# Rikorose/DeepFilterNet

Hardware: NVIDIA H100
Metric: 48kHz audio-sec/sec (batched enhance) (higher is better)
Workload: dtype f32 (bf16x3 tensor-core contractions, fp32 accumulate; DSP and gates IEEE fp32)

## Files before the change

deepfilternet_b200/csrc/dfb_ptx.cuh:

```cuda
#pragma once
#include <cuda.h>
#include <cuda_bf16.h>
#include <stdint.h>

namespace dfb {

__device__ __forceinline__ uint32_t smem_u32(const void *p) { return (uint32_t)__cvta_generic_to_shared(p); }

__device__ __forceinline__ void mbar_init(uint64_t *bar, uint32_t count) {
    asm volatile("mbarrier.init.shared::cta.b64 [%0], %1;" ::"r"(smem_u32(bar)), "r"(count));
}

__device__ __forceinline__ void mbar_expect_tx(uint64_t *bar, uint32_t bytes) {
    asm volatile("mbarrier.arrive.expect_tx.shared::cta.b64 _, [%0], %1;" ::"r"(smem_u32(bar)), "r"(bytes) : "memory");
}

__device__ __forceinline__ void mbar_wait(uint64_t *bar, uint32_t parity) {
    asm volatile(
        "{\n\t"
        ".reg .pred p;\n\t"
        "WAIT_%=:\n\t"
        "mbarrier.try_wait.parity.shared::cta.b64 p, [%0], %1;\n\t"
        "@p bra DONE_%=;\n\t"
        "bra WAIT_%=;\n\t"
// ... 46 lines not shown
__device__ __forceinline__ void warp_mma_sw128_k64(uint32_t a_hi, uint32_t a_lo, uint32_t b_hi, uint32_t b_lo, int m0, int n0,
                                                   float (&acc)[MT][8][4]) {
    const int lane = threadIdx.x & 31, mat = lane >> 3, rr = lane & 7;
#pragma unroll
    for (int ks = 0; ks < 4; ks++) {
        uint32_t ah[MT][4], al[MT][4];
#pragma unroll
        for (int mt = 0; mt < MT; mt++) {
            const int r = m0 + 16 * mt + rr + ((mat & 1) << 3);
            const uint32_t o = sw128_off(r, 2 * ks + (mat >> 1));
            ldsm_x4(a_hi + o, ah[mt]);
            ldsm_x4(a_lo + o, al[mt]);
        }
#pragma unroll
        for (int np = 0; np < 4; np++) {
            const int n = n0 + 16 * np + rr + ((mat >> 1) << 3);
            const uint32_t o = sw128_off(n, 2 * ks + (mat & 1));
            uint32_t bh[4], bl[4];
            ldsm_x4(b_hi + o, bh);
            ldsm_x4(b_lo + o, bl);
#pragma unroll
            for (int mt = 0; mt < MT; mt++) {
                mma_bf16x3(acc[mt][2 * np], ah[mt], al[mt], bh[0], bh[1], bl[0], bl[1]);
                mma_bf16x3(acc[mt][2 * np + 1], ah[mt], al[mt], bh[2], bh[3], bl[2], bl[3]);
            }
        }
    }
}

__device__ __forceinline__ void mbar_arrive(uint64_t *bar) {
    asm volatile("mbarrier.arrive.shared::cta.b64 _, [%0];" ::"r"(smem_u32(bar)) : "memory");
}



__device__ __forceinline__ void bf16x2_split(float x0, float x1, uint32_t &hi, uint32_t &lo) {
    __nv_bfloat162 h = __floats2bfloat162_rn(x0, x1);
    const float2 hf = __bfloat1622float2(h);
    __nv_bfloat162 l = __floats2bfloat162_rn(x0 - hf.x, x1 - hf.y);
    hi = *reinterpret_cast<uint32_t *>(&h);
    lo = *reinterpret_cast<uint32_t *>(&l);
}

__device__ __forceinline__ float4 lds128(uint32_t a) {
    float4 v;
    asm volatile("ld.shared.v4.f32 {%0, %1, %2, %3}, [%4];" : "=f"(v.x), "=f"(v.y), "=f"(v.z), "=f"(v.w) : "r"(a));
    return v;
}

__device__ __forceinline__ void sts128(uint32_t a, float4 v) {
    asm volatile("st.shared.v4.f32 [%0], {%1, %2, %3, %4};" ::"r"(a), "f"(v.x), "f"(v.y), "f"(v.z), "f"(v.w) : "memory");
}

__device__ __forceinline__ void sts64(uint32_t a, uint32_t x, uint32_t y) {
    asm volatile("st.shared.v2.b32 [%0], {%1, %2};" ::"r"(a), "r"(x), "r"(y) : "memory");
}

__device__ __forceinline__ uint32_t lds32(uint32_t a) {
    uint32_t v;
    asm volatile("ld.shared.b32 %0, [%1];" : "=r"(v) : "r"(a));
    return v;
}

__device__ __forceinline__ void mbar_init_a(uint32_t bar, uint32_t count) {
    asm volatile("mbarrier.init.shared::cta.b64 [%0], %1;" ::"r"(bar), "r"(count));
}
// ... 64 lines not shown
```

deepfilternet_b200/csrc/dfb_tc.cu:

```cuda
#include <cooperative_groups.h>
#include <atomic>
#include <map>
#include <mutex>
#include <cuda.h>
#include <cuda_bf16.h>

#include "dfb_common.cuh"
#include "dfb_dwpw.cuh"
#include "dfb_ptx.cuh"

namespace dfb {

constexpr int kBxBM = 128, kBxBN = 128, kBxBK = 64, kBxStages = 3, kBxThreads = 288;
constexpr int kBxBox = 128 * 128;

struct BxSmem {
    alignas(1024) unsigned char x[kBxStages][2][kBxBox];
    alignas(1024) unsigned char w[kBxStages][2][kBxBox];
    alignas(8) uint64_t full[kBxStages];
    uint64_t empty[kBxStages];
};

__global__ void __launch_bounds__(kBxThreads, 1)
k_gemm_bf16x3(const __grid_constant__ CUtensorMap tmXhi, const __grid_constant__ CUtensorMap tmXlo,
              const __grid_constant__ CUtensorMap tmWhi, const __grid_constant__ CUtensorMap tmWlo,
              const float *__restrict__ bias, float *__restrict__ Y, int64_t ldy, int M, int K, int nslices) {
    extern __shared__ __align__(1024) unsigned char tc_smem_raw[];
    BxSmem &sm = *reinterpret_cast<BxSmem *>(((uintptr_t)tc_smem_raw + 1023) & ~uintptr_t(1023));
    const int warp = threadIdx.x >> 5, lane = threadIdx.x & 31;
    const int n0 = (int)(blockIdx.x % nslices) * kBxBN, m0 = (int)(blockIdx.x / nslices) * kBxBM;
    const int nkb = K / kBxBK;
    if (threadIdx.x == 0) {
        for (int s = 0; s < kBxStages; s++) { mbar_init(&sm.full[s], 1); mbar_init(&sm.empty[s], 8); }
        fence_barrier_init();
    }
    __syncthreads();
    if (warp == 8) {
        if (lane == 0) {
            tma_prefetch_desc(&tmXhi); tma_prefetch_desc(&tmXlo); tma_prefetch_desc(&tmWhi); tma_prefetch_desc(&tmWlo);
            for (int kb = 0; kb < nkb; kb++) {
                const int s = kb % kBxStages, n = kb / kBxStages;
                if (n > 0) mbar_wait(&sm.empty[s], (n - 1) & 1);
                mbar_expect_tx(&sm.full[s], 4 * kBxBox);
                tma_load_2d(sm.x[s][0], &tmXhi, kb * kBxBK, m0, &sm.full[s]);
                tma_load_2d(sm.x[s][1], &tmXlo, kb * kBxBK, m0, &sm.full[s]);
                tma_load_2d(sm.w[s][0], &tmWhi, kb * kBxBK, n0, &sm.full[s]);
                tma_load_2d(sm.w[s][1], &tmWlo, kb * kBxBK, n0, &sm.full[s]);
            }
        }
        return;
    }
    const int wm = (warp & 3) * 32, wn = (warp >> 2) * 64;
    float acc[2][8][4];
#pragma unroll
    for (int a = 0; a < 2; a++)
#pragma unroll
        for (int b = 0; b < 8; b++)
#pragma unroll
            for (int c = 0; c < 4; c++) acc[a][b][c] = 0.f;
    for (int kb = 0; kb < nkb; kb++) {
        const int s = kb % kBxStages;
        mbar_wait(&sm.full[s], (kb / kBxStages) & 1);
        warp_mma_sw128_k64<2>(smem_u32(sm.x[s][0]), smem_u32(sm.x[s][1]), smem_u32(sm.w[s][0]), smem_u32(sm.w[s][1]), wm, wn, acc);
        __syncwarp();
        if (lane == 0) mbar_arrive(&sm.empty[s]);
    }
#pragma unroll
    for (int nt = 0; nt < 8; nt++) {
        const int n = n0 + wn + 8 * nt + 2 * (lane & 3);
        const float2 bn = bias ? make_float2(__ldg(bias + n), __ldg(bias + n + 1)) : make_float2(0.f, 0.f);
#pragma unroll
        for (int mt = 0; mt < 2; mt++)
#pragma unroll
            for (int h = 0; h < 2; h++) {
                const int m = m0 + wm + 16 * mt + (lane >> 2) + 8 * h;
                if (m < M)
                    *reinterpret_cast<float2 *>(Y + (int64_t)m * ldy + n) =
                        make_float2(acc[mt][nt][2 * h] + bn.x, acc[mt][nt][2 * h + 1] + bn.y);
            }
    }
}

constexpr int kDxThreads = 256;
constexpr uint32_t kDxW = 32768, kDxRaw = 49152, kDxTail = 64 * 4 + 32;


template <int MODE, int KT, int PATH, int MASK>
__global__ void __launch_bounds__(kDxThreads, 2)
k_dwpw_bx(DwPwParams p, const float *__restrict__ w_sw ) {
    extern __shared__ __align__(1024) unsigned char tc_smem_raw[];
    const uint32_t sb = smem_u32(tc_smem_raw);
    if (sb & 1023u) __trap();
    const int tid = threadIdx.x, warp = tid >> 5, lane = tid & 31;
    const int b = blockIdx.y, t0 = blockIdx.x * p.NF;
    const int nf = min(p.NF, p.T - t0);
    const int R = nf * p.Fout;
    const int tq0 = t0 - (KT - 1);
    const uint32_t fbytes = (uint32_t)p.Fin * kCh * 4;
    const uint32_t raw_in = sb + kDxRaw, raw_path = raw_in + (uint32_t)(p.NF + KT - 1) * fbytes;
    const uint32_t raw_e0 = raw_in + (uint32_t)(p.NF + KT - 1) * fbytes * (PATH ? 2u : 1u);
    const uint32_t obytes = (uint32_t)p.Fout * kCh * 4;
    const uint32_t tail = raw_e0 + (MASK ? (uint32_t)p.NF * obytes : 0u);
    const uint32_t s_bias = tail, bar_raw = tail + 264;
    const uint32_t s_mask = raw_in;
    if (tid == 0) {
        mbar_init_a(bar_raw, 1);
        fence_barrier_init();
        const int ta = max(tq0, 0), tb = t0 + nf;
        mbar_expect_tx_a(bar_raw, (uint32_t)(tb - ta) * fbytes * (PATH ? 2u : 1u) + 2u * kCh * 128u + (MASK ? (uint32_t)nf * obytes : 0u));
        if (MASK)
            for (int t = t0; t < tb; t++)
                bulk_load(raw_e0 + (uint32_t)(t - t0) * obytes, p.mk_e0 + ((int64_t)b * p.T + t) * p.Fout * kCh, obytes, bar_raw);
// ... 672 lines not shown
        if (rc) return rc;
    }
    if (xg == 0 || xg == 1) {
        if (H == 512 && ns == 16) return xg ? launch_gru_tc_n<16, 512, 1>(s, p) : launch_gru_tc_n<16, 512, 0>(s, p);
        if (H == 256 && ns == 16) return xg ? launch_gru_tc_n<16, 256, 1>(s, p) : launch_gru_tc_n<16, 256, 0>(s, p);
        if (H == 256 && ns == 32) return xg ? launch_gru_tc_n<32, 256, 1>(s, p) : launch_gru_tc_n<32, 256, 0>(s, p);
        if (H == 256 && ns == 48 && xg) return launch_gru_tc_n<48, 256, 1>(s, p);
    }
    return fail(DFB_ERR_UNSUPPORTED, "tensor-core recurrence: instance NS %d H %d XG %d is not built", ns, H, xg);
}

int cached_map_f32_sw128(CUtensorMap *out, const void *base, int64_t rows, int64_t cols, int64_t ld, int box_rows);

int launch_df_convp_tc(cudaStream_t s, const float *c0, const float *w_sw, const float *w2, const float *bias, float *coefs, int B, int T,
                       int Fd, const int64_t *first, int64_t w0) {
    if ((int64_t)B * T >= (int64_t(1) << 31) - 256 || B > 65535) return fail(DFB_ERR_UNSUPPORTED, "df pathway conv: batch too large for one launch");
    CUtensorMap mc;
    int rc;
    if ((rc = cached_map_f32_sw128(&mc, c0, (int64_t)B * T, (int64_t)Fd * kCh, (int64_t)Fd * kCh, 128))) return rc;
    const int smem = 1024 + (int)kCvTail + 512 + 64;
    static PerDeviceOnce attr_once;
    if (auto once_guard = attr_once.first())
        DFB_CUDA(cudaFuncSetAttribute(k_df_convp_tc<5, 5>, cudaFuncAttributeMaxDynamicSharedMemorySize, smem));
    CvParams p{w_sw, w2, bias, coefs, T, Fd, first, w0};
    dim3 grid((unsigned)((Fd + kCvBins - 1) / kCvBins), (unsigned)((T + kCvOut - 1) / kCvOut), (unsigned)B);
    DFB_PROF("k_df_convp_tc", s);
    k_df_convp_tc<5, 5><<<grid, kCvThreads, smem, s>>>(mc, p);
    DFB_LAUNCH_CHECK();
    return DFB_OK;
}

int cached_map_bf16(CUtensorMap *out, const void *base, int64_t rows, int64_t cols, int64_t ld, int box_rows);

int launch_gemm_bf16x3(cudaStream_t s, const void *x_hi, const void *x_lo, int64_t ldx, const void *w_hi, const void *w_lo,
                       const float *bias, float *y, int64_t ldy, int64_t M, int N, int K) {
    if (N % kBxBN || K % kBxBK || (ldx % 8) || M <= 0 || ldy % 2 || ((uintptr_t)w_hi & 15) || ((uintptr_t)w_lo & 15))
        return fail(DFB_ERR_UNSUPPORTED, "bf16x3 GEMM shape M=%lld N=%d K=%d", (long long)M, N, K);
    const int nslices = N / kBxBN;
    const int64_t ntiles = (M + kBxBM - 1) / kBxBM;
    if (ntiles * nslices > 0x7fffffff) return fail(DFB_ERR_UNSUPPORTED, "bf16x3 GEMM: M = %lld", (long long)M);
    CUtensorMap mxh, mxl, mwh, mwl;
    int rc;
    if ((rc = cached_map_bf16(&mxh, x_hi, M, K, ldx, kBxBM)) || (rc = cached_map_bf16(&mxl, x_lo, M, K, ldx, kBxBM)) ||
        (rc = cached_map_bf16(&mwh, w_hi, N, K, K, kBxBN)) || (rc = cached_map_bf16(&mwl, w_lo, N, K, K, kBxBN)))
        return rc;
    static PerDeviceOnce attr_once;
    const int smem = (int)sizeof(BxSmem) + 1024;
    if (auto once_guard = attr_once.first()) DFB_CUDA(cudaFuncSetAttribute(k_gemm_bf16x3, cudaFuncAttributeMaxDynamicSharedMemorySize, smem));
    DFB_PROF("k_gemm_bf16x3[gru_proj]", s);
    k_gemm_bf16x3<<<(unsigned)(ntiles * nslices), kBxThreads, smem, s>>>(mxh, mxl, mwh, mwl, bias, y, ldy, (int)M, K, nslices);
    DFB_LAUNCH_CHECK();
    return DFB_OK;
}

}

extern "C" int dfb_debug_gru_tc(const float *xproj, const float *whh, const float *bhh, const float *res, float *hout,
                                void *hout_hi, void *hout_lo, int planes_res, const float *h0, float *hT, const int64_t *first,
                                int64_t w0, int t0, int Ts, int B, int T, int H, int ns, int xg, void *stream) {
    if (!xproj || !whh || !bhh || (!hout && !hout_hi) || (!hout_hi != !hout_lo))
        return dfb::fail(DFB_ERR_INVALID, "gru_tc: null argument");
    if (B <= 0 || T <= 0 || t0 < 0 || (int64_t)t0 + T > Ts)
        return dfb::fail(DFB_ERR_INVALID, "gru_tc: B %d, window [%d, %d + %d) of %d frames", B, t0, t0, T, Ts);
    const dfb::GruWindow w{h0, hT, t0, Ts, first, w0};
    return dfb::launch_gru_tc((cudaStream_t)stream, xproj, whh, bhh, res, hout, (unsigned short *)hout_hi,
                              (unsigned short *)hout_lo, B, T, nullptr, 0, planes_res, &w, H, ns, xg);
}

extern "C" int dfb_debug_gemm_bf16x3(const void *x_hi, const void *x_lo, int64_t ldx, const void *w_hi, const void *w_lo,
                                     const float *bias, float *y, int64_t ldy, int64_t M, int N, int K, void *stream) {
    if (!x_hi || !x_lo || !w_hi || !w_lo || !y) return dfb::fail(DFB_ERR_INVALID, "gemm_bf16x3: null argument");
    return dfb::launch_gemm_bf16x3((cudaStream_t)stream, x_hi, x_lo, ldx, w_hi, w_lo, bias, y, ldy, M, N, K);
}
```

deepfilternet_b200/csrc/dfb_gl.cu:

```cuda
#include <cuda.h>
#include <cuda_bf16.h>

#include <map>
#include <mutex>
#include <tuple>

#include "dfb_common.cuh"
#include "dfb_dwpw.cuh"
#include "dfb_ptx.cuh"

namespace dfb {

constexpr int kGxThreads = 288, kGxMaxStages = 6, kGxBoxBytes = 128 * 128 ;
constexpr int kGxMaxChunks = 16;

struct GlBxParams {
    const unsigned short *w_img;
    const float *res; int64_t ldr;
    float *y; int64_t ldy;
    unsigned short *y_hi, *y_lo; int64_t ldp;
    int M, G, Ig, Hg, Hgp, gpc, act, stages;
    float oscale, ooffset;
    int stage_y;
};

__device__ __forceinline__ float gx_act(float x, int act) {
    if (act == 1) return fmaxf(x, 0.f);
    if (act == 2) return gt_tanh(x);
    return x;
}

__device__ __noinline__ void gl_store_chunk(const GlBxParams &p, int c, int g0, int cpg, int64_t mrow, int lane, uint32_t st,
                                            float a00, float a01, float a02, float a03, float a10, float a11, float a12, float a13) {
    const float a[2][4] = {{a00, a01, a02, a03}, {a10, a11, a12, a13}};
    const int gl = c / cpg;
    if (st) {
        const uint32_t pitch = (uint32_t)(p.gpc * p.Hg) * 4u;
#pragma unroll
        for (int j = 0; j < 2; j++) {
            const int n = (c - gl * cpg) * 16 + j * 8 + 2 * (lane & 3);
            if (n >= p.Hg) continue;
            const int lcol = gl * p.Hg + n;
            const int64_t col = (int64_t)g0 * p.Hg + lcol;
#pragma unroll
            for (int h = 0; h < 2; h++) {
                const uint32_t sa = st + (uint32_t)((lane >> 2) + 8 * h) * pitch + (uint32_t)lcol * 4u;
                float2 rv = make_float2(0.f, 0.f);
                if (p.res) asm volatile("ld.shared.v2.f32 {%0, %1}, [%2];" : "=f"(rv.x), "=f"(rv.y) : "r"(sa));
                float2 x;
                x.x = gx_act(a[j][2 * h], p.act) * p.oscale + p.ooffset + rv.x;
                x.y = gx_act(a[j][2 * h + 1], p.act) * p.oscale + p.ooffset + rv.y;
                sts64(sa, __float_as_uint(x.x), __float_as_uint(x.y));
                const int64_t m = mrow + 8 * h;
                if (p.y_hi && m < p.M) {
                    uint32_t hv, lv;
                    bf16x2_split(x.x, x.y, hv, lv);
                    *reinterpret_cast<uint32_t *>(p.y_hi + m * p.ldp + col) = hv;
                    *reinterpret_cast<uint32_t *>(p.y_lo + m * p.ldp + col) = lv;
                }
            }
        }
        return;
    }
#pragma unroll
    for (int j = 0; j < 2; j++) {
        const int n = (c - gl * cpg) * 16 + j * 8 + 2 * (lane & 3);
        if (n >= p.Hg) continue;
        const int64_t col = (int64_t)(g0 + gl) * p.Hg + n;
        float2 rv[2];
#pragma unroll
        for (int h = 0; h < 2; h++) {
            const int64_t m = mrow + 8 * h;
            rv[h] = (p.res && m < p.M) ? *reinterpret_cast<const float2 *>(p.res + m * p.ldr + col) : make_float2(0.f, 0.f);
        }
#pragma unroll
        for (int h = 0; h < 2; h++) {
            const int64_t m = mrow + 8 * h;
            if (m >= p.M) continue;
            float2 x;
            x.x = gx_act(a[j][2 * h], p.act) * p.oscale + p.ooffset + rv[h].x;
            x.y = gx_act(a[j][2 * h + 1], p.act) * p.oscale + p.ooffset + rv[h].y;
            if (p.y) *reinterpret_cast<float2 *>(p.y + m * p.ldy + col) = x;
            if (p.y_hi) {
                uint32_t hv, lv;
                bf16x2_split(x.x, x.y, hv, lv);
                *reinterpret_cast<uint32_t *>(p.y_hi + m * p.ldp + col) = hv;
                *reinterpret_cast<uint32_t *>(p.y_lo + m * p.ldp + col) = lv;
            }
        }
    }
}

__global__ void __launch_bounds__(kGxThreads, 1)
k_gl_bx(const __grid_constant__ CUtensorMap tmXhi, const __grid_constant__ CUtensorMap tmXlo, const __grid_constant__ CUtensorMap tmY,
        const __grid_constant__ CUtensorMap tmR, const __grid_constant__ GlBxParams p) {
    extern __shared__ __align__(1024) unsigned char gx_smem_raw[];
    const uint32_t sb = (smem_u32(gx_smem_raw) + 1023u) & ~1023u;
    const int warp = threadIdx.x >> 5, lane = threadIdx.x & 31;
    const int slice = blockIdx.x, g0 = slice * p.gpc;
    const int nch = p.gpc * p.Hgp / 16;
    const int cpg = p.Hgp / 16;
    const int nboxes = p.gpc * p.Ig / 64;
    const int ntiles = (p.M + 127) / 128;
    const uint32_t gbytes = (uint32_t)p.Ig * p.Hgp * 2;
    const uint32_t wplane = gbytes * p.gpc;
    const uint32_t lbo = (uint32_t)(p.Hgp / 8) * 128u;
    const uint32_t s_x = sb;
    const uint32_t s_w = s_x + (uint32_t)p.stages * 2 * kGxBoxBytes;
    const uint32_t ybox = 16u * (uint32_t)(p.gpc * p.Hg) * 4u;
    const uint32_t s_y = s_w + 2 * wplane;
    const uint32_t s_bar = (s_y + (p.stage_y ? 8 * ybox : 0u) + 127u) & ~127u;
    const uint32_t b_full = s_bar, b_empty = s_bar + 8 * kGxMaxStages, b_w = b_empty + 8 * kGxMaxStages;
    const uint32_t b_rfull = b_w + 8, b_rempty = b_rfull + 8 * 8;
    const bool res_tma = p.stage_y && p.res;
    if (threadIdx.x == 0) {
        for (int s = 0; s < p.stages; s++) { mbar_init_a(b_full + 8 * s, 1); mbar_init_a(b_empty + 8 * s, 8); }
        mbar_init_a(b_w, 1);
        for (int w = 0; w < 8; w++) { mbar_init_a(b_rfull + 8 * w, 1); mbar_init_a(b_rempty + 8 * w, 1); }
        fence_barrier_init();
        mbar_expect_tx_a(b_w, 2 * wplane);
        const unsigned char *src = reinterpret_cast<const unsigned char *>(p.w_img);
        bulk_load(s_w, src + (size_t)g0 * gbytes, wplane, b_w);
        bulk_load(s_w + wplane, src + (size_t)p.G * gbytes + (size_t)g0 * gbytes, wplane, b_w);
    }
    __syncthreads();
    if (warp == 8) {
        if (lane == 0) {
            tma_prefetch_desc(&tmXhi); tma_prefetch_desc(&tmXlo);
            if (res_tma) tma_prefetch_desc(&tmR);
            const int col0 = g0 * p.Ig;
            int it = 0, ti = 0;
            for (int tile = blockIdx.y; tile < ntiles; tile += gridDim.y, ti++) {
                for (int b = 0; b < nboxes; b++, it++) {
                    const int s = it % p.stages, n = it / p.stages;
                    if (n > 0) mbar_wait_a(b_empty + 8 * s, (uint32_t)((n - 1) & 1));
                    mbar_expect_tx_a(b_full + 8 * s, 2 * kGxBoxBytes);
                    const uint32_t dst = s_x + (uint32_t)s * 2 * kGxBoxBytes;
                    asm volatile(
                        "cp.async.bulk.tensor.2d.shared::cluster.global.mbarrier::complete_tx::bytes [%0], [%1, {%2, %3}], [%4];"
                        ::"r"(dst), "l"((uint64_t)&tmXhi), "r"(col0 + b * 64), "r"(tile * 128), "r"(b_full + 8 * s) : "memory");
                    asm volatile(
                        "cp.async.bulk.tensor.2d.shared::cluster.global.mbarrier::complete_tx::bytes [%0], [%1, {%2, %3}], [%4];"
                        ::"r"(dst + kGxBoxBytes), "l"((uint64_t)&tmXlo), "r"(col0 + b * 64), "r"(tile * 128), "r"(b_full + 8 * s) : "memory");
                }
                for (int w = 0; res_tma && w < 8; w++) {
                    if (ti > 0) mbar_wait_a(b_rempty + 8 * w, (uint32_t)((ti - 1) & 1));
                    mbar_expect_tx_a(b_rfull + 8 * w, ybox);
                    asm volatile(
                        "cp.async.bulk.tensor.2d.shared::cluster.global.mbarrier::complete_tx::bytes [%0], [%1, {%2, %3}], [%4];"
                        ::"r"(s_y + (uint32_t)w * ybox), "l"((uint64_t)&tmR), "r"(g0 * p.Hg), "r"(tile * 128 + 16 * w), "r"(b_rfull + 8 * w)
                        : "memory");
                }
            }
        }
        return;
    }
    const int mat = lane >> 3, rr = lane & 7;
    mbar_wait_a(b_w, 0);
    const uint32_t st = p.stage_y ? s_y + (uint32_t)warp * ybox : 0u;
    int it = 0, ti = 0;
    for (int tile = blockIdx.y; tile < ntiles; tile += gridDim.y, ti++) {
        float acc[kGxMaxChunks][2][4];
#pragma unroll
        for (int c = 0; c < kGxMaxChunks; c++)
#pragma unroll
            for (int e = 0; e < 8; e++) acc[c][e >> 2][e & 3] = 0.f;
        for (int b = 0; b < nboxes; b++, it++) {
            const int s = it % p.stages, n = it / p.stages;
            mbar_wait_a(b_full + 8 * s, (uint32_t)(n & 1));
            const uint32_t xs = s_x + (uint32_t)s * 2 * kGxBoxBytes;
#pragma unroll 1
            for (int k = 0; k < 4; k++) {
                const int col = b * 64 + k * 16;
                const int gl = col / p.Ig, kk = (col - gl * p.Ig) >> 4;
                uint32_t ah[4], al[4];
                const int r = warp * 16 + rr + ((mat & 1) << 3);
                ldsm_x4(xs + sw128_off(r, 2 * k + (mat >> 1)), ah);
                ldsm_x4(xs + kGxBoxBytes + sw128_off(r, 2 * k + (mat >> 1)), al);
                const uint32_t wa = s_w + (uint32_t)gl * gbytes + (uint32_t)(2 * kk + (mat & 1)) * lbo + (uint32_t)rr * 16u;
#pragma unroll
                for (int c = 0; c < kGxMaxChunks; c++) {
                    const int cg = c - gl * cpg;
                    if (c >= nch || cg < 0 || cg >= cpg) continue;
                    const uint32_t o = wa + (uint32_t)(2 * cg + (mat >> 1)) * 128u;
                    uint32_t bh[4], bl[4];
                    ldsm_x4(o, bh);
                    ldsm_x4(o + wplane, bl);
                    mma_bf16x3(acc[c][0], ah, al, bh[0], bh[1], bl[0], bl[1]);
                    mma_bf16x3(acc[c][1], ah, al, bh[2], bh[3], bl[2], bl[3]);
                }
            }
            __syncwarp();
            if (lane == 0) mbar_arrive_a(b_empty + 8 * s);
        }
        const int64_t mrow = (int64_t)tile * 128 + warp * 16 + (lane >> 2);
        if (res_tma) mbar_wait_a(b_rfull + 8 * warp, (uint32_t)(ti & 1));
#pragma unroll
        for (int c = 0; c < kGxMaxChunks; c++)
            if (c < nch)
                gl_store_chunk(p, c, g0, cpg, mrow, lane, st, acc[c][0][0], acc[c][0][1], acc[c][0][2], acc[c][0][3], acc[c][1][0],
                               acc[c][1][1], acc[c][1][2], acc[c][1][3]);
        if (st) {
            fence_proxy_async();
            __syncwarp();
            if (lane == 0) {
                asm volatile("cp.async.bulk.tensor.2d.global.shared::cta.bulk_group [%0, {%1, %2}], [%3];"
                             ::"l"((uint64_t)&tmY), "r"(g0 * p.Hg), "r"(tile * 128 + warp * 16), "r"(st) : "memory");
                asm volatile("cp.async.bulk.commit_group;" ::: "memory");
                asm volatile("cp.async.bulk.wait_group.read 0;" ::: "memory");
                if (res_tma) mbar_arrive_a(b_rempty + 8 * warp);
            }
            __syncwarp();
        }
    }
}

constexpr int kDeThreads = 288, kDeMaxStages = 6, kDeMaxChunks = 4;
constexpr uint32_t kDeBin = 32768;

struct DfEmbParams {
    const float *dw;
    const float *bias;
    const float *pw_sw;
    const unsigned short *w_img;
    const float *res; int64_t ldr;
    unsigned short *y_hi, *y_lo; int64_t ldp;
    int M, T, G, Ig, Hg, Hgp, S, stages;
    float oscale, ooffset;
    const int64_t *first;
    int64_t w0;
};

template <int KT>
__global__ void __launch_bounds__(kDeThreads, 1)
k_dwpw_gl(const __grid_constant__ CUtensorMap tmC0, const __grid_constant__ DfEmbParams p) {
    extern __shared__ __align__(1024) unsigned char de_smem_raw[];
    const uint32_t sb = (smem_u32(de_smem_raw) + 1023u) & ~1023u;
    const int warp = threadIdx.x >> 5, lane = threadIdx.x & 31;
    constexpr int RT = 128 - (KT - 1);
    const int ntiles = (p.M + RT - 1) / RT;
    const int j0 = blockIdx.x * p.S;
    const int f_lo = j0 > 0 ? 2 * j0 - 1 : 0, f_hi = 2 * (j0 + p.S);
    const int gps = p.S * kCh / p.Ig, cpg = p.Hgp / 16, nch = gps * cpg;
    const int g0 = j0 * kCh / p.Ig;
    const uint32_t gbytes = (uint32_t)p.Ig * p.Hgp * 2;
    const uint32_t wplane = gbytes * gps;
    const uint32_t lbo = (uint32_t)(p.Hgp / 8) * 128u;
// ... 314 lines not shown
bool gl_bx_geometry(int G, int Ig, int Hg, int *gpc_out, int *hgp_out, int *stages_out) {
    if (Ig % 16 || Hg % 4 || G < 1) return false;
    const int Hgp = (Hg + 15) / 16 * 16;
    if (Hgp > 256) return false;
    int best = 0;
    for (int gpc = 1; gpc <= G; gpc++) {
        if (G % gpc) continue;
        if (gpc * Hgp > 256 || (gpc * Hgp) % 32) continue;
        if ((gpc * Ig) % 64) continue;
        if ((size_t)gpc * Ig * Hgp * 4 > 100 * 1024) continue;
        best = gpc;
    }
    if (!best) return false;
    const int w = best * Ig * Hgp * 4;
    int stages = (227 * 1024 - 2048 - w - 256) / (2 * kGxBoxBytes);
    if (stages > kGxMaxStages) stages = kGxMaxStages;
    if (stages < 2) return false;
    *gpc_out = best; *hgp_out = Hgp; *stages_out = stages;
    return true;
}

int launch_gl_bx(cudaStream_t s, const unsigned short *x_hi, const unsigned short *x_lo, int64_t ldx, const float *w_img,
                 const float *res, int64_t ldr, float *y, int64_t ldy, unsigned short *y_hi, unsigned short *y_lo, int64_t ldp,
                 int64_t M, int G, int Ig, int Hg, int act, float oscale, float ooffset) {
    int gpc = 0, Hgp = 0, stages = 0;
    if (!gl_bx_geometry(G, Ig, Hg, &gpc, &Hgp, &stages) || M <= 0 || M > 0x7fffffff || (ldx % 8) || ((uintptr_t)x_hi & 15) ||
        ((uintptr_t)x_lo & 15) || (y && ((ldy % 4) || ((uintptr_t)y & 15))) || (res && ((ldr % 4) || ((uintptr_t)res & 15))) ||
        (y_hi && ((ldp % 4) || ((uintptr_t)y_hi & 7) || ((uintptr_t)y_lo & 7))))
        return DFB_ERR_UNSUPPORTED;
    CUtensorMap mh, ml;
    int rc;
    if ((rc = cached_map_bf16(&mh, x_hi, M, (int64_t)G * Ig, ldx, 128)) || (rc = cached_map_bf16(&ml, x_lo, M, (int64_t)G * Ig, ldx, 128)))
        return rc;
    const int wbytes = gpc * Ig * Hgp * 4, ybytes = 128 * gpc * Hg * 4;
    int stages_y = (227 * 1024 - 2048 - wbytes - ybytes - 256) / (2 * kGxBoxBytes);
    if (stages_y > kGxMaxStages) stages_y = kGxMaxStages;
    const bool stage_y = y && stages_y >= 2;
    CUtensorMap my = mh, mr = mh;
    if (stage_y) {
        stages = stages_y;
        if ((rc = cached_map_f32_rows(&my, y, M, (int64_t)G * Hg, ldy, gpc * Hg, 16))) return rc;
        if (res && (rc = cached_map_f32_rows(&mr, res, M, (int64_t)G * Hg, ldr, gpc * Hg, 16))) return rc;
    }
    GlBxParams p{reinterpret_cast<const unsigned short *>(w_img), res, ldr, y, ldy, y_hi, y_lo, ldp,
                 (int)M, G, Ig, Hg, Hgp, gpc, act, stages, oscale, ooffset, stage_y ? 1 : 0};
    const int smem = 1024 + stages * 2 * kGxBoxBytes + wbytes + (stage_y ? ybytes : 0) + 128 + 256;
    static PerDeviceOnce attr_once;
    if (auto once_guard = attr_once.first())
        DFB_CUDA(cudaFuncSetAttribute(k_gl_bx, cudaFuncAttributeMaxDynamicSharedMemorySize, 227 * 1024));
    int dev = 0, sms = 0;
    DFB_CUDA(cudaGetDevice(&dev));
    DFB_CUDA(cudaDeviceGetAttribute(&sms, cudaDevAttrMultiProcessorCount, dev));
    const int slices = G / gpc, ntiles = (int)((M + 127) / 128);
    int groups = sms / slices;
    if (groups < 1) groups = 1;
    if (groups > ntiles) groups = ntiles;
    DFB_PROF("k_gl_bx", s);
    k_gl_bx<<<dim3((unsigned)slices, (unsigned)groups), kGxThreads, smem, s>>>(mh, ml, my, mr, p);
    DFB_LAUNCH_CHECK();
    return DFB_OK;
}

}

extern "C" int dfb_debug_gl_bx(const void *x_hi, const void *x_lo, int64_t ldx, const float *w_img, const float *res, int64_t ldr,
                               float *y, int64_t ldy, void *y_hi, void *y_lo, int64_t ldp, int64_t M, int G, int Ig, int Hg,
                               int act, float oscale, float ooffset, void *stream) {
    if (!x_hi || !x_lo || !w_img || (!y && !y_hi) || (!y_hi != !y_lo)) return dfb::fail(DFB_ERR_INVALID, "gl_bx: null argument");
    const int r = dfb::launch_gl_bx((cudaStream_t)stream, (const unsigned short *)x_hi, (const unsigned short *)x_lo, ldx, w_img, res,
                                    ldr, y, ldy, (unsigned short *)y_hi, (unsigned short *)y_lo, ldp, M, G, Ig, Hg, act, oscale, ooffset);
    if (r == DFB_ERR_UNSUPPORTED) return dfb::fail(r, "gl_bx: shape G %d Ig %d Hg %d or pointer alignment not built", G, Ig, Hg);
    return r;
}

namespace dfb {

bool df_emb_geometry(int Fd, int G, int Ig, int Hg, int kt, int *s_out, int *stages_out) {
    if ((kt != 1 && kt != 2) || Fd % 2 || Ig % 16 || Hg % 4 || G < 1 || G * Ig != Fd / 2 * kCh) return false;
    int S = 1;
    while ((S * kCh) % Ig) S++;
    const int Hgp = (Hg + 15) / 16 * 16;
    if ((Fd / 2) % S || (S * kCh / Ig) * (Hgp / 16) > kDeMaxChunks) return false;
    const int fixed = 1024 + 2 * kCh * 128 + S * kCh * Hgp * 4 + 256 + kt * 3 * kCh * 4 + 128 + 2 * 8 * kDeMaxStages + 8;
    int stages = (227 * 1024 - fixed) / (int)kDeBin;
    if (stages > kDeMaxStages) stages = kDeMaxStages;
    if (stages < 3) return false;
    *s_out = S; *stages_out = stages;
    return true;
}

int launch_df_emb(cudaStream_t s, const float *c0, int64_t M, int T, int Fd, int kt, const float *dw, const float *bias,
// ... 36 lines not shown
```

Measured before the change: 69360.

## Rewrite bf16x3 GRU projection GEMM as persistent warp-specialized WGMMA kernel

```diff
diff --git a/deepfilternet_b200/csrc/dfb_ptx.cuh b/deepfilternet_b200/csrc/dfb_ptx.cuh
--- a/deepfilternet_b200/csrc/dfb_ptx.cuh
+++ b/deepfilternet_b200/csrc/dfb_ptx.cuh
@@ -102,6 +102,44 @@
     asm volatile("mbarrier.arrive.shared::cta.b64 _, [%0];" ::"r"(smem_u32(bar)) : "memory");
 }
 
+__device__ __forceinline__ uint64_t wgmma_desc_sw128(uint32_t saddr) {
+    return (uint64_t)((saddr & 0x3FFFFu) >> 4) | ((uint64_t)1 << 16) | ((uint64_t)(1024 >> 4) << 32) | ((uint64_t)1 << 62);
+}
+
+__device__ __forceinline__ void wgmma_fence() { asm volatile("wgmma.fence.sync.aligned;" ::: "memory"); }
+__device__ __forceinline__ void wgmma_commit() { asm volatile("wgmma.commit_group.sync.aligned;" ::: "memory"); }
+template <int N>
+__device__ __forceinline__ void wgmma_wait() {
+    asm volatile("wgmma.wait_group.sync.aligned %0;" ::"n"(N) : "memory");
+}
+
+__device__ __forceinline__ void wgmma_fence_operand(float &r) { asm volatile("" : "+f"(r)::"memory"); }
+
+__device__ __forceinline__ void wgmma_m64n128k16_bf16(float (&d)[64], uint64_t desc_a, uint64_t desc_b, uint32_t scale_d) {
+    asm volatile(
+        "{\n\t.reg .pred p;\n\tsetp.ne.b32 p, %66, 0;\n\t"
+        "wgmma.mma_async.sync.aligned.m64n128k16.f32.bf16.bf16 "
+        "{%0, %1, %2, %3, %4, %5, %6, %7, %8, %9, %10, %11, %12, %13, %14, %15, "
+        "%16, %17, %18, %19, %20, %21, %22, %23, %24, %25, %26, %27, %28, %29, %30, %31, "
+        "%32, %33, %34, %35, %36, %37, %38, %39, %40, %41, %42, %43, %44, %45, %46, %47, "
+        "%48, %49, %50, %51, %52, %53, %54, %55, %56, %57, %58, %59, %60, %61, %62, %63}, "
+        "%64, %65, p, 1, 1, 0, 0;\n\t}\n"
+        : "+f"(d[0]), "+f"(d[1]), "+f"(d[2]), "+f"(d[3]), "+f"(d[4]), "+f"(d[5]), "+f"(d[6]), "+f"(d[7]),
+          "+f"(d[8]), "+f"(d[9]), "+f"(d[10]), "+f"(d[11]), "+f"(d[12]), "+f"(d[13]), "+f"(d[14]), "+f"(d[15]),
+          "+f"(d[16]), "+f"(d[17]), "+f"(d[18]), "+f"(d[19]), "+f"(d[20]), "+f"(d[21]), "+f"(d[22]), "+f"(d[23]),
+          "+f"(d[24]), "+f"(d[25]), "+f"(d[26]), "+f"(d[27]), "+f"(d[28]), "+f"(d[29]), "+f"(d[30]), "+f"(d[31]),
+          "+f"(d[32]), "+f"(d[33]), "+f"(d[34]), "+f"(d[35]), "+f"(d[36]), "+f"(d[37]), "+f"(d[38]), "+f"(d[39]),
+          "+f"(d[40]), "+f"(d[41]), "+f"(d[42]), "+f"(d[43]), "+f"(d[44]), "+f"(d[45]), "+f"(d[46]), "+f"(d[47]),
+          "+f"(d[48]), "+f"(d[49]), "+f"(d[50]), "+f"(d[51]), "+f"(d[52]), "+f"(d[53]), "+f"(d[54]), "+f"(d[55]),
+          "+f"(d[56]), "+f"(d[57]), "+f"(d[58]), "+f"(d[59]), "+f"(d[60]), "+f"(d[61]), "+f"(d[62]), "+f"(d[63])
+        : "l"(desc_a), "l"(desc_b), "r"(scale_d));
+}
+
+template <int R>
+__device__ __forceinline__ void setmaxnreg_dec() { asm volatile("setmaxnreg.dec.sync.aligned.u32 %0;" ::"n"(R)); }
+template <int R>
+__device__ __forceinline__ void setmaxnreg_inc() { asm volatile("setmaxnreg.inc.sync.aligned.u32 %0;" ::"n"(R)); }
+
 
 
 __device__ __forceinline__ void bf16x2_split(float x0, float x1, uint32_t &hi, uint32_t &lo) {
diff --git a/deepfilternet_b200/csrc/dfb_tc.cu b/deepfilternet_b200/csrc/dfb_tc.cu
--- a/deepfilternet_b200/csrc/dfb_tc.cu
+++ b/deepfilternet_b200/csrc/dfb_tc.cu
@@ -11,7 +11,8 @@
 
 namespace dfb {
 
-constexpr int kBxBM = 128, kBxBN = 128, kBxBK = 64, kBxStages = 3, kBxThreads = 288;
+constexpr int kBxBM = 128, kBxBN = 128, kBxBK = 64, kBxStages = 3, kBxThreads = 384;
+constexpr int kBxTileRing = 8;
 constexpr int kBxBox = 128 * 128;
 
 struct BxSmem {
@@ -19,65 +20,123 @@
     alignas(1024) unsigned char w[kBxStages][2][kBxBox];
     alignas(8) uint64_t full[kBxStages];
     uint64_t empty[kBxStages];
+    uint64_t turn[2];
+    uint64_t tile_full[kBxTileRing];
+    int tile_id[kBxTileRing];
 };
 
 __global__ void __launch_bounds__(kBxThreads, 1)
 k_gemm_bf16x3(const __grid_constant__ CUtensorMap tmXhi, const __grid_constant__ CUtensorMap tmXlo,
               const __grid_constant__ CUtensorMap tmWhi, const __grid_constant__ CUtensorMap tmWlo,
-              const float *__restrict__ bias, float *__restrict__ Y, int64_t ldy, int M, int K, int nslices) {
+              const float *__restrict__ bias, float *__restrict__ Y, int64_t ldy, int M, int K, int nslices, int ntiles,
+              unsigned *__restrict__ sched ) {
     extern __shared__ __align__(1024) unsigned char tc_smem_raw[];
     BxSmem &sm = *reinterpret_cast<BxSmem *>(((uintptr_t)tc_smem_raw + 1023) & ~uintptr_t(1023));
-    const int warp = threadIdx.x >> 5, lane = threadIdx.x & 31;
-    const int n0 = (int)(blockIdx.x % nslices) * kBxBN, m0 = (int)(blockIdx.x / nslices) * kBxBM;
+    const int wg = threadIdx.x >> 7;
     const int nkb = K / kBxBK;
     if (threadIdx.x == 0) {
-        for (int s = 0; s < kBxStages; s++) { mbar_init(&sm.full[s], 1); mbar_init(&sm.empty[s], 8); }
+        for (int s = 0; s < kBxStages; s++) { mbar_init(&sm.full[s], 1); mbar_init(&sm.empty[s], 4); }
+        mbar_init(&sm.turn[0], 1);
+        mbar_init(&sm.turn[1], 1);
+        for (int r = 0; r < kBxTileRing; r++) mbar_init(&sm.tile_full[r], 1);
         fence_barrier_init();
     }
     __syncthreads();
-    if (warp == 8) {
-        if (lane == 0) {
+    if (wg == 0) {
+        setmaxnreg_dec<40>();
+        if (threadIdx.x == 0) {
             tma_prefetch_desc(&tmXhi); tma_prefetch_desc(&tmXlo); tma_prefetch_desc(&tmWhi); tma_prefetch_desc(&tmWlo);
-            for (int kb = 0; kb < nkb; kb++) {
-                const int s = kb % kBxStages, n = kb / kBxStages;
-                if (n > 0) mbar_wait(&sm.empty[s], (n - 1) & 1);
-                mbar_expect_tx(&sm.full[s], 4 * kBxBox);
-                tma_load_2d(sm.x[s][0], &tmXhi, kb * kBxBK, m0, &sm.full[s]);
-                tma_load_2d(sm.x[s][1], &tmXlo, kb * kBxBK, m0, &sm.full[s]);
-                tma_load_2d(sm.w[s][0], &tmWhi, kb * kBxBK, n0, &sm.full[s]);
-                tma_load_2d(sm.w[s][1], &tmWlo, kb * kBxBK, n0, &sm.full[s]);
+            int it = 0;
+            for (int j = 0;; j++) {
+                const int tile = (int)atomicAdd(sched, 1u);
+                sm.tile_id[j % kBxTileRing] = tile < ntiles ? tile : -1;
+                mbar_arrive(&sm.tile_full[j % kBxTileRing]);
+                if (tile >= ntiles) {
+                    sm.tile_id[(j + 1) % kBxTileRing] = -1;
+                    mbar_arrive(&sm.tile_full[(j + 1) % kBxTileRing]);
+                    break;
+                }
+                const int m0 = (tile / nslices) * kBxBM, n0 = (tile % nslices) * kBxBN;
+                for (int kb = 0; kb < nkb; kb++, it++) {
+                    const int s = it % kBxStages, n = it / kBxStages;
+                    if (n > 0) mbar_wait(&sm.empty[s], (n - 1) & 1);
+                    mbar_expect_tx(&sm.full[s], 4 * kBxBox);
+                    tma_load_2d(sm.x[s][0], &tmXhi, kb * kBxBK, m0, &sm.full[s]);
+                    tma_load_2d(sm.x[s][1], &tmXlo, kb * kBxBK, m0, &sm.full[s]);
+                    tma_load_2d(sm.w[s][0], &tmWhi, kb * kBxBK, n0, &sm.full[s]);
+                    tma_load_2d(sm.w[s][1], &tmWlo, kb * kBxBK, n0, &sm.full[s]);
+                }
+            }
+            __threadfence();
+            if (atomicAdd(sched + 1, 1u) == gridDim.x - 1) {
+                atomicExch(sched, 0u);
+                atomicExch(sched + 1, 0u);
             }
         }
         return;
     }
-    const int wm = (warp & 3) * 32, wn = (warp >> 2) * 64;
-    float acc[2][8][4];
-#pragma unroll
-    for (int a = 0; a < 2; a++)
-#pragma unroll
-        for (int b = 0; b < 8; b++)
-#pragma unroll
-            for (int c = 0; c < 4; c++) acc[a][b][c] = 0.f;
-    for (int kb = 0; kb < nkb; kb++) {
-        const int s = kb % kBxStages;
-        mbar_wait(&sm.full[s], (kb / kBxStages) & 1);
-        warp_mma_sw128_k64<2>(smem_u32(sm.x[s][0]), smem_u32(sm.x[s][1]), smem_u32(sm.w[s][0]), smem_u32(sm.w[s][1]), wm, wn, acc);
-        __syncwarp();
-        if (lane == 0) mbar_arrive(&sm.empty[s]);
-    }
-#pragma unroll
-    for (int nt = 0; nt < 8; nt++) {
-        const int n = n0 + wn + 8 * nt + 2 * (lane & 3);
-        const float2 bn = bias ? make_float2(__ldg(bias + n), __ldg(bias + n + 1)) : make_float2(0.f, 0.f);
-#pragma unroll
-        for (int mt = 0; mt < 2; mt++)
-#pragma unroll
-            for (int h = 0; h < 2; h++) {
-                const int m = m0 + wm + 16 * mt + (lane >> 2) + 8 * h;
-                if (m < M)
-                    *reinterpret_cast<float2 *>(Y + (int64_t)m * ldy + n) =
-                        make_float2(acc[mt][nt][2 * h] + bn.x, acc[mt][nt][2 * h + 1] + bn.y);
-            }
+    setmaxnreg_inc<232>();
+    const int c = wg - 1, warp = (threadIdx.x >> 5) & 3, lane = threadIdx.x & 31;
+    float acc[2][64];
+#pragma unroll
+    for (int h = 0; h < 2; h++)
+#pragma unroll
+        for (int i = 0; i < 64; i++) acc[h][i] = 0.f;
+    for (int j = c;; j += 2) {
+        mbar_wait(&sm.tile_full[j % kBxTileRing], (uint32_t)(j / kBxTileRing) & 1);
+        const int tile = *(volatile int *)&sm.tile_id[j % kBxTileRing];
+        if (tile < 0) break;
+        const int m0 = (tile / nslices) * kBxBM, n0 = (tile % nslices) * kBxBN;
+        if (j > 0) mbar_wait(&sm.turn[c], (uint32_t)((j - 2 + c) / 2) & 1);
+        int it = j * nkb;
+        for (int kb = 0; kb < nkb; kb++, it++) {
+            const int s = it % kBxStages;
+            mbar_wait(&sm.full[s], (it / kBxStages) & 1);
+            if (kb == nkb - 1 && (threadIdx.x & 127) == 0) mbar_arrive(&sm.turn[c ^ 1]);
+#pragma unroll
+            for (int h = 0; h < 2; h++)
+#pragma unroll
+                for (int i = 0; i < 64; i++) wgmma_fence_operand(acc[h][i]);
+            wgmma_fence();
+            const uint32_t xh = smem_u32(sm.x[s][0]), xl = smem_u32(sm.x[s][1]);
+            const uint32_t wh = smem_u32(sm.w[s][0]), wl = smem_u32(sm.w[s][1]);
+#pragma unroll
+            for (int ks = 0; ks < kBxBK / 16; ks++) {
+                const uint64_t dwh = wgmma_desc_sw128(wh + 32 * ks), dwl = wgmma_desc_sw128(wl + 32 * ks);
+#pragma unroll
+                for (int h = 0; h < 2; h++) {
+                    const uint64_t dxh = wgmma_desc_sw128(xh + 8192 * h + 32 * ks), dxl = wgmma_desc_sw128(xl + 8192 * h + 32 * ks);
+                    wgmma_m64n128k16_bf16(acc[h], dxh, dwh, (kb | ks) != 0);
+                    wgmma_m64n128k16_bf16(acc[h], dxl, dwh, 1);
+                    wgmma_m64n128k16_bf16(acc[h], dxh, dwl, 1);
+                }
+            }
+            wgmma_commit();
+            if (kb > 0) {
+                wgmma_wait<1>();
+                if (lane == 0) mbar_arrive(&sm.empty[(it - 1) % kBxStages]);
+            }
+        }
+        wgmma_wait<0>();
+#pragma unroll
+        for (int h = 0; h < 2; h++)
+#pragma unroll
+            for (int i = 0; i < 64; i++) wgmma_fence_operand(acc[h][i]);
+        if (lane == 0) mbar_arrive(&sm.empty[(it - 1) % kBxStages]);
+#pragma unroll
+        for (int q = 0; q < 16; q++) {
+            const int n = n0 + 8 * q + 2 * (lane & 3);
+            const float2 bn = bias ? make_float2(__ldg(bias + n), __ldg(bias + n + 1)) : make_float2(0.f, 0.f);
+#pragma unroll
+            for (int h = 0; h < 2; h++)
+#pragma unroll
+                for (int e = 0; e < 2; e++) {
+                    const int m = m0 + 64 * h + 16 * warp + (lane >> 2) + 8 * e;
+                    if (m < M)
+                        __stcs(reinterpret_cast<float2 *>(Y + (int64_t)m * ldy + n),
+                               make_float2(acc[h][4 * q + 2 * e] + bn.x, acc[h][4 * q + 2 * e + 1] + bn.y));
+                }
+        }
     }
 }
 
@@ -816,13 +875,29 @@
 
 int cached_map_bf16(CUtensorMap *out, const void *base, int64_t rows, int64_t cols, int64_t ld, int box_rows);
 
+static unsigned *gemm_sched(cudaStream_t s) {
+    static std::mutex mu;
+    static std::map<std::pair<int, cudaStream_t>, unsigned *> pool;
+    int dev = 0;
+    cudaGetDevice(&dev);
+    std::lock_guard<std::mutex> lk(mu);
+    unsigned *&p = pool[{dev, s}];
+    if (!p) {
+        if (cudaMalloc(&p, 2 * sizeof(unsigned)) != cudaSuccess || cudaMemsetAsync(p, 0, 2 * sizeof(unsigned), s) != cudaSuccess) {
+            if (p) cudaFree(p);
+            p = nullptr;
+        }
+    }
+    return p;
+}
+
 int launch_gemm_bf16x3(cudaStream_t s, const void *x_hi, const void *x_lo, int64_t ldx, const void *w_hi, const void *w_lo,
                        const float *bias, float *y, int64_t ldy, int64_t M, int N, int K) {
     if (N % kBxBN || K % kBxBK || (ldx % 8) || M <= 0 || ldy % 2 || ((uintptr_t)w_hi & 15) || ((uintptr_t)w_lo & 15))
         return fail(DFB_ERR_UNSUPPORTED, "bf16x3 GEMM shape M=%lld N=%d K=%d", (long long)M, N, K);
     const int nslices = N / kBxBN;
     const int64_t ntiles = (M + kBxBM - 1) / kBxBM;
-    if (ntiles * nslices > 0x7fffffff) return fail(DFB_ERR_UNSUPPORTED, "bf16x3 GEMM: M = %lld", (long long)M);
+    if (ntiles * nslices > 0x7fff0000) return fail(DFB_ERR_UNSUPPORTED, "bf16x3 GEMM: M = %lld", (long long)M);
     CUtensorMap mxh, mxl, mwh, mwl;
     int rc;
     if ((rc = cached_map_bf16(&mxh, x_hi, M, K, ldx, kBxBM)) || (rc = cached_map_bf16(&mxl, x_lo, M, K, ldx, kBxBM)) ||
@@ -831,8 +906,15 @@
     static PerDeviceOnce attr_once;
     const int smem = (int)sizeof(BxSmem) + 1024;
     if (auto once_guard = attr_once.first()) DFB_CUDA(cudaFuncSetAttribute(k_gemm_bf16x3, cudaFuncAttributeMaxDynamicSharedMemorySize, smem));
+    int dev = 0, sms = 0;
+    DFB_CUDA(cudaGetDevice(&dev));
+    DFB_CUDA(cudaDeviceGetAttribute(&sms, cudaDevAttrMultiProcessorCount, dev));
+    const int64_t tiles = ntiles * nslices;
+    const unsigned grid = (unsigned)(tiles < sms ? tiles : sms);
+    unsigned *sched = gemm_sched(s);
+    if (!sched) return fail(DFB_ERR_OOM, "bf16x3 GEMM tile counter");
     DFB_PROF("k_gemm_bf16x3[gru_proj]", s);
-    k_gemm_bf16x3<<<(unsigned)(ntiles * nslices), kBxThreads, smem, s>>>(mxh, mxl, mwh, mwl, bias, y, ldy, (int)M, K, nslices);
+    k_gemm_bf16x3<<<grid, kBxThreads, smem, s>>>(mxh, mxl, mwh, mwl, bias, y, ldy, (int)M, K, nslices, (int)tiles, sched);
     DFB_LAUNCH_CHECK();
     return DFB_OK;
 }
```

After: 71390, median of 6. 1.03x the previous value.

## Stage bf16 hi/lo output planes in shared memory and store via TMA

Applied to the files above, without the earlier changes.

```diff
diff --git a/deepfilternet_b200/csrc/dfb_gl.cu b/deepfilternet_b200/csrc/dfb_gl.cu
--- a/deepfilternet_b200/csrc/dfb_gl.cu
+++ b/deepfilternet_b200/csrc/dfb_gl.cu
@@ -13,6 +13,8 @@
 
 constexpr int kGxThreads = 288, kGxMaxStages = 6, kGxBoxBytes = 128 * 128 ;
 constexpr int kGxMaxChunks = 16;
+constexpr uint32_t kGxPlaneBlockBytes = 4096;
+constexpr uint32_t kGxPlaneWarpBytes = 2 * kGxPlaneBlockBytes;
 
 struct GlBxParams {
     const unsigned short *w_img;
@@ -22,12 +24,43 @@
     int M, G, Ig, Hg, Hgp, gpc, act, stages;
     float oscale, ooffset;
     int stage_y;
+    int stage_p;
 };
 
 __device__ __forceinline__ float gx_act(float x, int act) {
     if (act == 1) return fmaxf(x, 0.f);
     if (act == 2) return gt_tanh(x);
     return x;
+}
+
+__device__ __forceinline__ void gl_stage_planes(uint32_t sp, int c, int r, int cc, float x0, float x1) {
+    uint32_t hv, lv;
+    bf16x2_split(x0, x1, hv, lv);
+    const uint32_t o = sw128_off(r, 2 * (c & 3) + (cc >> 3)) + (uint32_t)(cc & 7) * 2u;
+    asm volatile("st.shared.b32 [%0], %1;" ::"r"(sp + o), "r"(hv) : "memory");
+    asm volatile("st.shared.b32 [%0], %1;" ::"r"(sp + 2048u + o), "r"(lv) : "memory");
+}
+
+__device__ __noinline__ void gl_stage_chunk(const GlBxParams &p, int c, uint32_t st, uint32_t sp, float a00, float a01, float a02,
+                                            float a03, float a10, float a11, float a12, float a13) {
+    const float a[2][4] = {{a00, a01, a02, a03}, {a10, a11, a12, a13}};
+    const int lane = threadIdx.x & 31;
+    const uint32_t pitch = (uint32_t)(p.gpc * p.Hg) * 4u;
+#pragma unroll
+    for (int j = 0; j < 2; j++) {
+        const int cc = j * 8 + 2 * (lane & 3);
+#pragma unroll
+        for (int h = 0; h < 2; h++) {
+            const uint32_t sa = st + (uint32_t)((lane >> 2) + 8 * h) * pitch + (uint32_t)(16 * c + cc) * 4u;
+            float2 rv = make_float2(0.f, 0.f);
+            if (st && p.res) asm volatile("ld.shared.v2.f32 {%0, %1}, [%2];" : "=f"(rv.x), "=f"(rv.y) : "r"(sa));
+            float2 x;
+            x.x = gx_act(a[j][2 * h], p.act) * p.oscale + p.ooffset + rv.x;
+            x.y = gx_act(a[j][2 * h + 1], p.act) * p.oscale + p.ooffset + rv.y;
+            if (st) sts64(sa, __float_as_uint(x.x), __float_as_uint(x.y));
+            gl_stage_planes(sp, c, (lane >> 2) + 8 * h, cc, x.x, x.y);
+        }
+    }
 }
 
 __device__ __noinline__ void gl_store_chunk(const GlBxParams &p, int c, int g0, int cpg, int64_t mrow, int lane, uint32_t st,
@@ -93,7 +126,8 @@
 
 __global__ void __launch_bounds__(kGxThreads, 1)
 k_gl_bx(const __grid_constant__ CUtensorMap tmXhi, const __grid_constant__ CUtensorMap tmXlo, const __grid_constant__ CUtensorMap tmY,
-        const __grid_constant__ CUtensorMap tmR, const __grid_constant__ GlBxParams p) {
+        const __grid_constant__ CUtensorMap tmR, const __grid_constant__ CUtensorMap tmPh, const __grid_constant__ CUtensorMap tmPl,
+        const __grid_constant__ GlBxParams p) {
     extern __shared__ __align__(1024) unsigned char gx_smem_raw[];
     const uint32_t sb = (smem_u32(gx_smem_raw) + 1023u) & ~1023u;
     const int warp = threadIdx.x >> 5, lane = threadIdx.x & 31;
@@ -109,7 +143,8 @@
     const uint32_t s_w = s_x + (uint32_t)p.stages * 2 * kGxBoxBytes;
     const uint32_t ybox = 16u * (uint32_t)(p.gpc * p.Hg) * 4u;
     const uint32_t s_y = s_w + 2 * wplane;
-    const uint32_t s_bar = (s_y + (p.stage_y ? 8 * ybox : 0u) + 127u) & ~127u;
+    const uint32_t s_p = s_y + (p.stage_y ? 8 * ybox : 0u);
+    const uint32_t s_bar = (s_p + (p.stage_p ? 8u * kGxPlaneWarpBytes : 0u) + 127u) & ~127u;
     const uint32_t b_full = s_bar, b_empty = s_bar + 8 * kGxMaxStages, b_w = b_empty + 8 * kGxMaxStages;
     const uint32_t b_rfull = b_w + 8, b_rempty = b_rfull + 8 * 8;
     const bool res_tma = p.stage_y && p.res;
@@ -158,6 +193,7 @@
     const int mat = lane >> 3, rr = lane & 7;
     mbar_wait_a(b_w, 0);
     const uint32_t st = p.stage_y ? s_y + (uint32_t)warp * ybox : 0u;
+    const uint32_t spw = p.stage_p ? s_p + (uint32_t)warp * kGxPlaneWarpBytes : 0u;
     int it = 0, ti = 0;
     for (int tile = blockIdx.y; tile < ntiles; tile += gridDim.y, ti++) {
         float acc[kGxMaxChunks][2][4];
@@ -196,10 +232,35 @@
         const int64_t mrow = (int64_t)tile * 128 + warp * 16 + (lane >> 2);
         if (res_tma) mbar_wait_a(b_rfull + 8 * warp, (uint32_t)(ti & 1));
 #pragma unroll
-        for (int c = 0; c < kGxMaxChunks; c++)
-            if (c < nch)
+        for (int c = 0; c < kGxMaxChunks; c++) {
+            if (c >= nch) continue;
+            const uint32_t sp = spw ? spw + (uint32_t)((c >> 2) & 1) * kGxPlaneBlockBytes : 0u;
+            if (sp) {
+                if ((c & 3) == 0) {
+                    if (lane == 0) asm volatile("cp.async.bulk.wait_group.read 1;" ::: "memory");
+                    __syncwarp();
+                }
+            }
+            if (sp)
+                gl_stage_chunk(p, c, st, sp, acc[c][0][0], acc[c][0][1], acc[c][0][2], acc[c][0][3], acc[c][1][0], acc[c][1][1],
+                               acc[c][1][2], acc[c][1][3]);
+            else
                 gl_store_chunk(p, c, g0, cpg, mrow, lane, st, acc[c][0][0], acc[c][0][1], acc[c][0][2], acc[c][0][3], acc[c][1][0],
                                acc[c][1][1], acc[c][1][2], acc[c][1][3]);
+            if (sp && (c & 3) == 3) {
+                fence_proxy_async();
+                __syncwarp();
+                if (lane == 0) {
+                    const int col = g0 * p.Hg + 16 * (c - 3), row = tile * 128 + warp * 16;
+                    asm volatile("cp.async.bulk.tensor.2d.global.shared::cta.bulk_group [%0, {%1, %2}], [%3];"
+                                 ::"l"((uint64_t)&tmPh), "r"(col), "r"(row), "r"(sp) : "memory");
+                    asm volatile("cp.async.bulk.tensor.2d.global.shared::cta.bulk_group [%0, {%1, %2}], [%3];"
+                                 ::"l"((uint64_t)&tmPl), "r"(col), "r"(row), "r"(sp + 2048u) : "memory");
+                    asm volatile("cp.async.bulk.commit_group;" ::: "memory");
+                    if (c + 1 == nch && (nch & 4)) asm volatile("cp.async.bulk.wait_group.read 0;" ::: "memory");
+                }
+            }
+        }
         if (st) {
             fence_proxy_async();
             __syncwarp();
@@ -213,6 +274,7 @@
             __syncwarp();
         }
     }
+    if (p.stage_p && lane == 0) asm volatile("cp.async.bulk.wait_group.read 0;" ::: "memory");
 }
 
 constexpr int kDeThreads = 288, kDeMaxStages = 6, kDeMaxChunks = 4;
@@ -593,19 +655,26 @@
     int rc;
     if ((rc = cached_map_bf16(&mh, x_hi, M, (int64_t)G * Ig, ldx, 128)) || (rc = cached_map_bf16(&ml, x_lo, M, (int64_t)G * Ig, ldx, 128)))
         return rc;
-    const int wbytes = gpc * Ig * Hgp * 4, ybytes = 128 * gpc * Hg * 4;
-    int stages_y = (227 * 1024 - 2048 - wbytes - ybytes - 256) / (2 * kGxBoxBytes);
-    if (stages_y > kGxMaxStages) stages_y = kGxMaxStages;
-    const bool stage_y = y && stages_y >= 2;
-    CUtensorMap my = mh, mr = mh;
+    const int wbytes = gpc * Ig * Hgp * 4, ybytes = 128 * gpc * Hg * 4, pbytes = 8 * (int)kGxPlaneWarpBytes;
+    auto ring = [&](int staged) {
+        const int s = (227 * 1024 - 2048 - wbytes - staged - 256) / (2 * kGxBoxBytes);
+        return s > kGxMaxStages ? kGxMaxStages : s;
+    };
+    const bool stage_y = y && ring(ybytes) >= 2;
+    const bool stage_p = y_hi && Hg % 16 == 0 && (gpc * Hg) % 64 == 0 && ldp % 8 == 0 && !((uintptr_t)y_hi & 15) &&
+                         !((uintptr_t)y_lo & 15) && (y ? stage_y : !res) && ring((stage_y ? ybytes : 0) + pbytes) >= 2;
+    CUtensorMap my = mh, mr = mh, mph = mh, mpl = mh;
     if (stage_y) {
-        stages = stages_y;
         if ((rc = cached_map_f32_rows(&my, y, M, (int64_t)G * Hg, ldy, gpc * Hg, 16))) return rc;
         if (res && (rc = cached_map_f32_rows(&mr, res, M, (int64_t)G * Hg, ldr, gpc * Hg, 16))) return rc;
     }
+    if (stage_p && ((rc = cached_map_bf16(&mph, y_hi, M, (int64_t)G * Hg, ldp, 16)) || (rc = cached_map_bf16(&mpl, y_lo, M, (int64_t)G * Hg, ldp, 16))))
+        return rc;
+    const int staged = (stage_y ? ybytes : 0) + (stage_p ? pbytes : 0);
+    if (staged) stages = ring(staged);
     GlBxParams p{reinterpret_cast<const unsigned short *>(w_img), res, ldr, y, ldy, y_hi, y_lo, ldp,
-                 (int)M, G, Ig, Hg, Hgp, gpc, act, stages, oscale, ooffset, stage_y ? 1 : 0};
-    const int smem = 1024 + stages * 2 * kGxBoxBytes + wbytes + (stage_y ? ybytes : 0) + 128 + 256;
+                 (int)M, G, Ig, Hg, Hgp, gpc, act, stages, oscale, ooffset, stage_y ? 1 : 0, stage_p ? 1 : 0};
+    const int smem = 1024 + stages * 2 * kGxBoxBytes + wbytes + staged + 128 + 256;
     static PerDeviceOnce attr_once;
     if (auto once_guard = attr_once.first())
         DFB_CUDA(cudaFuncSetAttribute(k_gl_bx, cudaFuncAttributeMaxDynamicSharedMemorySize, 227 * 1024));
@@ -617,7 +686,7 @@
     if (groups < 1) groups = 1;
     if (groups > ntiles) groups = ntiles;
     DFB_PROF("k_gl_bx", s);
-    k_gl_bx<<<dim3((unsigned)slices, (unsigned)groups), kGxThreads, smem, s>>>(mh, ml, my, mr, p);
+    k_gl_bx<<<dim3((unsigned)slices, (unsigned)groups), kGxThreads, smem, s>>>(mh, ml, my, mr, mph, mpl, p);
     DFB_LAUNCH_CHECK();
     return DFB_OK;
 }
```

Measured after the change: 69250 before, 71340 after, median of 6. 1.03x the previous value.
